# wooginawunan/multi-modal-uncertainty

Hardware: AMD Instinct MI355X
Metric: image+text samples/sec/node, MMBT Food-101 bs=256 seq=512; ECE/NLL parity (higher is better)
Workload: dtype bf16

## Files before the change

### multi-modal-uncertainty_amd/csrc/gemm.hip

```cpp
#include "mmu_common.h"
#include "mmu_internal.h"
#include <cstdlib>

namespace mmu {

constexpr int BKT = 64;

#ifdef MMU_GEMM_STAMPS
__device__ uint64_t g_gemm_stamps[1 << 16][4];
#define GEMM_STAMP(i)                                                                       \
  do {                                                                                      \
    if (threadIdx.x == 0) {                                                                 \
      const int lin_ = (int)(blockIdx.x + gridDim.x * (blockIdx.y + gridDim.y * blockIdx.z)); \
      if (lin_ < (1 << 16)) g_gemm_stamps[lin_][i] = __builtin_amdgcn_s_memtime();          \
    }                                                                                       \
  } while (0)
#else
#define GEMM_STAMP(i) \
  do {                \
  } while (0)
#endif

static __device__ __forceinline__ int sw_mn(int r) { return (r & 7) ^ (((r >> 3) & 1) << 2); }

static __device__ __forceinline__ void tile_of(int pid, int tiles_m, int tiles_n, int group_m, int& tm, int& tn) {
  const int per_group = group_m * tiles_n;
  const int g = pid / per_group, first = g * group_m;
  const int gm = tiles_m - first < group_m ? tiles_m - first : group_m;
  const int r = pid - g * per_group;
  tm = first + r % gm;
  tn = r / gm;
}
static __device__ __forceinline__ void block_tile(const GemmParams& p, int64_t& z, int& slice, int& tm, int& tn) {
  const int ntiles = p.tiles_m * p.tiles_n;
  const int per_z = ntiles * (int)gridDim.y;
  const int lin = (int)(blockIdx.x + gridDim.x * (blockIdx.y + gridDim.y * blockIdx.z));
  const int pid = xcd_remap(lin, per_z * (int)gridDim.z);
  z = pid / per_z;
  const int r = pid - (int)z * per_z;
  slice = r / ntiles;
  tile_of(r - slice * ntiles, p.tiles_m, p.tiles_n, p.group_m, tm, tn);
}

template <bool KMAJ, int ROWB>
static __device__ __forceinline__ bf16x8 s_frag(const char* s, int row0, int ks, int l) {
  if (KMAJ) {
    const int row = row0 + (l & 15), c = 4 * ks + (l >> 4);
    return *(const bf16x8*)(s + row * 128 + ((c ^ (row & 7)) << 4));
  } else {
    const int g = l >> 4, i = l & 15, q = i >> 2, p = i & 3;
    const int b = row0 >> 4;
    const int k0 = 32 * ks + 8 * g + q, k1 = k0 + 4;
    const char* a0 = s + k0 * ROWB + ((b ^ sw_mn(k0)) << 5) + 8 * p;
    const char* a1 = s + k1 * ROWB + ((b ^ sw_mn(k1)) << 5) + 8 * p;
    bf16x4 lo = __builtin_amdgcn_ds_read_tr16_b64_v4bf16((MMU_LDS(bf16x4)*)a0);
    bf16x4 hi = __builtin_amdgcn_ds_read_tr16_b64_v4bf16((MMU_LDS(bf16x4)*)a1);
    return __builtin_shufflevector(lo, hi, 0, 1, 2, 3, 4, 5, 6, 7);
  }
}


template <int EPI, bool OUT_F32>
static __device__ __forceinline__ void epi_oct(const GemmParams& p, void* cdst, bf16* xdst, uint64_t qd,
                                               float (&v)[8], const float (&in)[8], float scale, uint32_t thr,
                                               uint64_t seed) {
  if (EPI == MMU_EPI_BIAS_GELU) {
    float d[8];
#pragma unroll
    for (int r = 0; r < 8; ++r) gelu_pair(v[r], v[r], d[r]);
    if (xdst) {
      bf16x8 o;
#pragma unroll
      for (int r = 0; r < 8; ++r) o[r] = f2bf(d[r]);
      *(bf16x8*)xdst = o;
    }
  } else if (EPI == MMU_EPI_BIAS_DROP_RES) {
    if (thr) {
      const uint32_t keep = mmu_keep4(seed, qd, thr) | (mmu_keep4(seed, qd + 1, thr) << 4);
#pragma unroll
      for (int r = 0; r < 8; ++r) v[r] = ((keep >> r) & 1) ? v[r] * scale : 0.f;
    }
#pragma unroll
    for (int r = 0; r < 8; ++r) v[r] += in[r];
  } else if (EPI == MMU_EPI_BIAS_DROP_QGELU) {
    uint32_t keep = 0xFFu;
    if (thr) keep = mmu_keep4(seed, qd, thr) | (mmu_keep4(seed, qd + 1, thr) << 4);
    float d[8];
#pragma unroll
    for (int r = 0; r < 8; ++r) {
      const float kz = ((keep >> r) & 1) ? scale : 0.f;
      const float u = v[r] * kz;
      const float sg = __builtin_amdgcn_rcpf(1.0f + __builtin_amdgcn_exp2f(u * -2.4554669595930157f));
      v[r] = u * sg;
      d[r] = kz * fmaf(1.702f * u * sg, 1.0f - sg, sg);
    }
    if (xdst) {
      bf16x8 o;
#pragma unroll
      for (int r = 0; r < 8; ++r) o[r] = f2bf(d[r]);
      *(bf16x8*)xdst = o;
    }
  } else if (EPI == MMU_EPI_DGELU) {
#pragma unroll
    for (int r = 0; r < 8; ++r) v[r] *= in[r];
  } else if (EPI == MMU_EPI_ADD_RES) {
#pragma unroll
    for (int r = 0; r < 8; ++r) v[r] += in[r];
  }
  if (OUT_F32) {
    float4* C = (float4*)cdst;
    float4 lo = make_float4(v[0], v[1], v[2], v[3]), hi = make_float4(v[4], v[5], v[6], v[7]);
// ... 382 lines not shown
    const char* sb = sa + SBM * BKT * 2;
    const bool more = kt + 1 < nk;
    if (more) {
      const int64_t k1 = kb + (int64_t)(kt + 1) * BKT;
      conva_g_load(ra, p.A, p, cr, k1, t);
      g_load<true>(rb, p.B, p.ldb, n0, p.N, k1, ke, t);
    }
#pragma unroll
    for (int ks = 0; ks < 2; ++ks) {
      bf16x8 fb[4], fa[4];
#pragma unroll
      for (int i = 0; i < 4; ++i) fb[i] = s_frag<true, 256>(sb, 64 * wn + 16 * i, ks, l);
#pragma unroll
      for (int j = 0; j < 4; ++j) fa[j] = s_frag<true, 256>(sa, 64 * wm + 16 * j, ks, l);
#pragma unroll
      for (int i = 0; i < 4; ++i)
#pragma unroll
        for (int j = 0; j < 4; ++j)
          acc[i][j] = __builtin_amdgcn_mfma_f32_16x16x32_bf16(fb[i], fa[j], acc[i][j], 0, 0, 0);
    }
    if (more) {
      char* dst = smem + ((kt + 1) & 1) * S_STAGE;
      s_store<true>(dst, ra, t);
      s_store<true>(dst + SBM * BKT * 2, rb, t);
    }
    __syncthreads();
  }
  epilogue_block<EPI, false, 4>(p, z, slice, m0 + 64 * wm, n0 + 64 * wn, acc, l, smem + w * 16384);
}

constexpr int BBM = 256, BBN = 256;
constexpr int B_TILE = BBM * BKT * 2;
constexpr int B_STAGE = 2 * B_TILE;

template <bool KMAJ>
static __device__ __forceinline__ void dma_tile(char* s, __amdgpu_buffer_rsrc_t rsrc, int64_t ld, int64_t r0,
                                                int64_t k0, int w, int l) {
#pragma unroll
  for (int i = 0; i < 4; ++i) {
    const int piece = w * 4 + i;
    uint32_t src;
    if (KMAJ) {
      const int row = piece * 8 + (l >> 3), c = (l & 7) ^ (row & 7);
      src = (uint32_t)(((r0 + row) * ld + k0 + 8 * c) * 2);
    } else {
      const int kr = piece * 2 + (l >> 5), j = l & 31;
      const int b = (j >> 1) ^ sw_mn(kr);
      src = (uint32_t)(((k0 + kr) * ld + r0 + 16 * b + 8 * (j & 1)) * 2);
    }
    __builtin_amdgcn_raw_ptr_buffer_load_lds(rsrc, (MMU_LDS(void)*)(s + piece * 1024), 16, src, 0, 0, 0);
  }
}

static __device__ __forceinline__ void dma_tile_convb(char* s, __amdgpu_buffer_rsrc_t rsrc, const GemmParams& p,
                                                      int dh, int dw, int64_t ci0, int64_t k0, int w, int l) {
  const int H = p.conv_h, W = p.conv_w, C = p.conv_c, s_ = p.conv_s;
  const int Wo = p.conv_wo, HW = p.conv_ho * Wo;
  const float rhw = 1.0f / (float)HW, rw = 1.0f / (float)Wo;
#pragma unroll
  for (int i = 0; i < 4; ++i) {
    const int piece = w * 4 + i;
    const int kr = piece * 2 + (l >> 5), j = l & 31;
    const int b = (j >> 1) ^ sw_mn(kr);
    const int pix = (int)k0 + kr;
    int img = (int)((float)pix * rhw);
    int rem = pix - img * HW;
    if (rem < 0) { --img; rem += HW; } else if (rem >= HW) { ++img; rem -= HW; }
    int hh = (int)((float)rem * rw);
    int ww = rem - hh * Wo;
    if (ww < 0) { --hh; ww += Wo; } else if (ww >= Wo) { ++hh; ww -= Wo; }
    hh = hh * s_ + dh;
    ww = ww * s_ + dw;
    const bool ok = pix < p.K && (unsigned)hh < (unsigned)H && (unsigned)ww < (unsigned)W;
    const uint32_t src = ok ? (uint32_t)(((((int64_t)img * H + hh) * W + ww) * C + ci0 + 16 * b + 8 * (j & 1)) * 2)
                            : 0x7FFFFFF0u;
    __builtin_amdgcn_raw_ptr_buffer_load_lds(rsrc, (MMU_LDS(void)*)(s + piece * 1024), 16, src, 0, 0, 0);
  }
}

struct ConvRows {
  int base[4], h[4], w[4];
};
static __device__ __forceinline__ ConvRows conv_rows_init(const GemmParams& p, int64_t m0, int w, int l) {
  ConvRows r;
  const int Wo = p.conv_wo, HWo = p.conv_ho * Wo;
#pragma unroll
  for (int i = 0; i < 4; ++i) {
    const int row = (w * 4 + i) * 8 + (l >> 3);
    const int64_t pix = m0 + row;
    const int img = (int)(pix / HWo), rem = (int)(pix - (int64_t)img * HWo);
    const int ho = rem / Wo;
    r.base[i] = pix < p.M ? img * p.conv_h : -1;
    r.h[i] = ho * p.conv_s - p.conv_pad;
    r.w[i] = (rem - ho * Wo) * p.conv_s - p.conv_pad;
  }
  return r;
}
static __device__ __forceinline__ void dma_tile_conva(char* s, __amdgpu_buffer_rsrc_t rsrc, const GemmParams& p,
                                                      const ConvRows& r, int64_t k0, int w, int l) {
  const int H = p.conv_h, W = p.conv_w, C = p.conv_c;
  const int tap = (int)(k0 / C), ci0 = (int)(k0 - (int64_t)tap * C);
  const int dh = tap / p.conv_ks, dw = tap - dh * p.conv_ks;
#pragma unroll
  for (int i = 0; i < 4; ++i) {
    const int piece = w * 4 + i;
    const int row = piece * 8 + (l >> 3), c = (l & 7) ^ (row & 7);
    const int hh = r.h[i] + dh, ww = r.w[i] + dw;
    const bool ok = r.base[i] >= 0 && (unsigned)hh < (unsigned)H && (unsigned)ww < (unsigned)W && k0 < p.K;
    const uint32_t src = ok ? (uint32_t)((((int64_t)(r.base[i] + hh) * W + ww) * C + ci0 + 8 * c) * 2) : 0x7FFFFFF0u;
    __builtin_amdgcn_raw_ptr_buffer_load_lds(rsrc, (MMU_LDS(void)*)(s + piece * 1024), 16, src, 0, 0, 0);
  }
}

template <bool AK, bool BKM, int EPI, bool OUT_F32, int GATHER>
static __device__ __forceinline__ void gemm_big_body(const GemmParams& p) {
  __shared__ __attribute__((aligned(16))) char smem[2 * B_STAGE];
  const int t = threadIdx.x, l = t & 63;
  const int w = __builtin_amdgcn_readfirstlane(t >> 6);
  const int wm = w >> 2, wn = w & 3;
  int tm, tn, slice;
  int64_t z;
  GEMM_STAMP(0);
  block_tile(p, z, slice, tm, tn);
  const int64_t m0 = (int64_t)tm * BBM, n0 = (int64_t)tn * BBN;
  const int64_t a_bytes = GATHER == 2 ? p.conv_in_bytes : (AK ? p.M * p.lda : p.K * p.lda) * 2;
  const int64_t b_bytes = GATHER == 1 ? p.conv_in_bytes : (BKM ? p.N * p.ldb : p.K * p.ldb) * 2;
  const __amdgpu_buffer_rsrc_t ra =
      __builtin_amdgcn_make_buffer_rsrc((void*)(p.A + z * p.sA), 0, (int)(uint32_t)a_bytes, 0x00020000);
  const __amdgpu_buffer_rsrc_t rb =
      __builtin_amdgcn_make_buffer_rsrc((void*)(p.B + z * p.sB), 0, (int)(uint32_t)b_bytes, 0x00020000);

  f32x4 acc[4][8];
#pragma unroll
  for (int i = 0; i < 4; ++i)
#pragma unroll
    for (int j = 0; j < 8; ++j) acc[i][j] = f32x4{0.f, 0.f, 0.f, 0.f};

  const int64_t kb = (int64_t)slice * p.kchunk;
  const int64_t ke = kb + p.kchunk < p.K ? kb + p.kchunk : p.K;
  const int nk = (int)((ke - kb + BKT - 1) / BKT);
  const int tap = GATHER == 1 ? (int)(n0 / p.conv_c) : 0;
  const int dh = GATHER == 1 ? tap / p.conv_ks - p.conv_pad : 0;
  const int dw = GATHER == 1 ? tap % p.conv_ks - p.conv_pad : 0;
  const int64_t ci0 = GATHER == 1 ? n0 - (int64_t)tap * p.conv_c : 0;
  auto dma_b = [&](char* d, int64_t k) {
    if (GATHER == 1) dma_tile_convb(d, rb, p, dh, dw, ci0, k, w, l);
    else dma_tile<BKM>(d, rb, p.ldb, n0, k, w, l);
  };
  ConvRows crow;
  if (GATHER == 2) crow = conv_rows_init(p, m0, w, l);
  auto dma_a = [&](char* d, int64_t k) {
    if (GATHER == 2) dma_tile_conva(d, ra, p, crow, k, w, l);
    else dma_tile<AK>(d, ra, p.lda, m0, k, w, l);
  };
  dma_a(smem, kb);
  dma_b(smem + B_TILE, kb);
  asm volatile("s_waitcnt vmcnt(0)" ::: "memory");
  __syncthreads();
  GEMM_STAMP(1);
  for (int kt = 0; kt < nk; ++kt) {
    const char* sa = smem + (kt & 1) * B_STAGE;
    const char* sb = sa + B_TILE;
    if (kt + 1 < nk) {
      char* d = smem + ((kt + 1) & 1) * B_STAGE;
      const int64_t k1 = kb + (int64_t)(kt + 1) * BKT;
      dma_a(d, k1);
      dma_b(d + B_TILE, k1);
    }
#pragma unroll
    for (int ks = 0; ks < 2; ++ks) {
      bf16x8 fb[4], fa[8];
#pragma unroll
      for (int i = 0; i < 4; ++i) fb[i] = s_frag<BKM, 512>(sb, 64 * wn + 16 * i, ks, l);
#pragma unroll
      for (int j = 0; j < 8; ++j) fa[j] = s_frag<AK, 512>(sa, 128 * wm + 16 * j, ks, l);
#pragma unroll
      for (int i = 0; i < 4; ++i)
#pragma unroll
        for (int j = 0; j < 8; ++j)
          acc[i][j] = __builtin_amdgcn_mfma_f32_16x16x32_bf16(fb[i], fa[j], acc[i][j], 0, 0, 0);
    }
    asm volatile("s_waitcnt vmcnt(0)" ::: "memory");
    __syncthreads();
  }
  GEMM_STAMP(2);
  epilogue_block<EPI, OUT_F32, 8>(p, z, slice, m0 + 128 * wm, n0 + 64 * wn, acc, l, smem + w * 16384);
#ifdef MMU_GEMM_STAMPS
  asm volatile("s_waitcnt vmcnt(0)" ::: "memory");
#endif
  GEMM_STAMP(3);
}

template <bool AK, bool BKM, int EPI, bool OUT_F32>
__global__ __launch_bounds__(512) void gemm_big_kernel(GemmParams p) {
  gemm_big_body<AK, BKM, EPI, OUT_F32, 0>(p);
}

__global__ __launch_bounds__(512) void gemm_convw_kernel(GemmParams p) {
  gemm_big_body<false, false, MMU_EPI_STORE, true, 1>(p);
}

template <int EPI>
__global__ __launch_bounds__(512) void gemm_conva_kernel(GemmParams p) {
  gemm_big_body<true, true, EPI, false, 2>(p);
}

constexpr int WBM = 256, WBN = 384;
constexpr int W_TA = WBM * BKT * 2;
constexpr int W_TB = WBN * BKT * 2;
constexpr int W_STAGE = W_TA + W_TB;

template <int P>
static __device__ __forceinline__ void dma_kmaj(char* s, __amdgpu_buffer_rsrc_t rsrc, int64_t ld, int64_t r0,
                                                int64_t k0, int w, int l) {
#pragma unroll
  for (int i = 0; i < P; ++i) {
    const int piece = w * P + i;
    const int row = piece * 8 + (l >> 3), c = (l & 7) ^ (row & 7);
    const uint32_t src = (uint32_t)(((r0 + row) * ld + k0 + 8 * c) * 2);
    __builtin_amdgcn_raw_ptr_buffer_load_lds(rsrc, (MMU_LDS(void)*)(s + piece * 1024), 16, src, 0, 0, 0);
  }
}

template <int EPI, bool OUT_F32>
__global__ __launch_bounds__(512) void gemm_wide_kernel(GemmParams p) {
  __shared__ __attribute__((aligned(16))) char smem[2 * W_STAGE];
  const int t = threadIdx.x, l = t & 63;
  const int w = __builtin_amdgcn_readfirstlane(t >> 6);
  const int wm = w >> 1, wn = w & 1;
  int tm, tn, slice;
  int64_t z;
  block_tile(p, z, slice, tm, tn);
  const int64_t m0 = (int64_t)tm * WBM, n0 = (int64_t)tn * WBN;
  const __amdgpu_buffer_rsrc_t ra =
      __builtin_amdgcn_make_buffer_rsrc((void*)(p.A + z * p.sA), 0, (int)(uint32_t)(p.M * p.lda * 2), 0x00020000);
  const __amdgpu_buffer_rsrc_t rb =
      __builtin_amdgcn_make_buffer_rsrc((void*)(p.B + z * p.sB), 0, (int)(uint32_t)(p.N * p.ldb * 2), 0x00020000);
  f32x4 acc[3][4][4];
#pragma unroll
  for (int c = 0; c < 3; ++c)
#pragma unroll
    for (int i = 0; i < 4; ++i)
#pragma unroll
      for (int j = 0; j < 4; ++j) acc[c][i][j] = f32x4{0.f, 0.f, 0.f, 0.f};
  const int nk = (int)(p.K / BKT);
  dma_kmaj<4>(smem, ra, p.lda, m0, 0, w, l);
  dma_kmaj<6>(smem + W_TA, rb, p.ldb, n0, 0, w, l);
  asm volatile("s_waitcnt vmcnt(0)" ::: "memory");
  __syncthreads();
  for (int kt = 0; kt < nk; ++kt) {
    const char* sa = smem + (kt & 1) * W_STAGE;
// ... 541 lines not shown
```

### multi-modal-uncertainty_amd/csrc/attention.hip

```cpp
#include "mmu_common.h"
#include "mmu_internal.h"
#include <cstdlib>
#include <type_traits>
#include <utility>

namespace mmu {

constexpr float LOG2E = 1.4426950408889634f;
constexpr float LN2 = 0.6931471805599453f;
constexpr float NEG_INF = -__builtin_huge_valf();

static __device__ __forceinline__ uint32_t lowbias32(uint32_t x) {
  x ^= x >> 16; x *= 0x7feb352du; x ^= x >> 15; x *= 0x846ca68bu; x ^= x >> 16;
  return x;
}
static __device__ __forceinline__ uint32_t seed_for(uint64_t seed, int bh) {
  return lowbias32((uint32_t)seed ^ lowbias32((uint32_t)(seed >> 32) + 0x9E3779B9u * (uint32_t)(bh + 1)));
}
static __device__ __forceinline__ uint32_t drop_pair(uint32_t sbh, uint32_t q, uint32_t key, uint32_t Lp) {
  return lowbias32(((q * Lp + key) >> 1) ^ sbh);
}

static __device__ __forceinline__ float max3f(float a, float b, float c) {
  return __builtin_fmaxf(__builtin_fmaxf(a, b), c);
}
static __device__ __forceinline__ uint32_t bfi(uint32_t m, uint32_t a, uint32_t b) {
  return (m & a) | (~m & b);
}
static __device__ __forceinline__ uint32_t keepmask(uint32_t w, uint32_t pos) {
  uint32_t r;
  asm("v_bfe_i32 %0, %1, %2, 1" : "=v"(r) : "v"(w), "v"(pos));
  return r;
}
template <typename F, int... R>
static __device__ __forceinline__ void static_for(F&& f, std::integer_sequence<int, R...>) {
  (f(std::integral_constant<int, R>{}), ...);
}
template <int POS>
static __device__ __forceinline__ uint32_t keepmask(uint32_t w) {
  uint32_t r;
  asm("v_bfe_i32 %0, %1, %2, 1" : "=v"(r) : "v"(w), "n"(POS));
  return r;
}
static __host__ __device__ __forceinline__ uint32_t drop_thr(float p) { return (uint32_t)(p * 65536.0f + 0.5f); }

static __device__ __forceinline__ int fsw(int r) { return (((r >> 1) & 1) << 2) | ((r >> 3) & 3); }
static __device__ __forceinline__ int tile_off(int row, int chunk) { return row * 128 + ((chunk ^ fsw(row)) << 4); }

static __device__ __forceinline__ bf16x8 row_frag(const char* s, int row0, int ks, int l) {
  return *(const bf16x8*)(s + tile_off(row0 + (l & 31), 2 * ks + (l >> 5)));
}
static __device__ __forceinline__ bf16x8 tr_frag(const char* s, int row0, int col0, int l) {
  const int g = l >> 4, i = l & 15, q = i >> 2, p = i & 3, h = g >> 1;
  const int col = col0 + 16 * (g & 1) + 4 * p;
  const int r0 = row0 + 4 * h + q, r1 = r0 + 8;
  const int cb = col * 2;
  const char* a0 = s + tile_off(r0, cb >> 4) + (cb & 15);
  const char* a1 = s + tile_off(r1, cb >> 4) + (cb & 15);
  bf16x4 lo = __builtin_amdgcn_ds_read_tr16_b64_v4bf16((MMU_LDS(bf16x4)*)a0);
  bf16x4 hi = __builtin_amdgcn_ds_read_tr16_b64_v4bf16((MMU_LDS(bf16x4)*)a1);
  return __builtin_shufflevector(lo, hi, 0, 1, 2, 3, 4, 5, 6, 7);
}
static __device__ __forceinline__ bf16x8 acc_frag(const f32x16& a, int s) {
  bf16x8 r;
#pragma unroll
  for (int j = 0; j < 8; ++j) r[j] = f2bf(a[8 * s + j]);
  return r;
}
static __device__ __forceinline__ bf16x8 scale_frag(uint4 u, float sc) {
  bf16x8 v = *(bf16x8*)&u;
#pragma unroll
  for (int j = 0; j < 8; ++j) v[j] = f2bf(bf2f(v[j]) * sc);
  return v;
}

static __device__ __forceinline__ __amdgpu_buffer_rsrc_t urs(const void* base, int bytes) {
  const uint64_t a = (uint64_t)base;
  const uint32_t lo = __builtin_amdgcn_readfirstlane((uint32_t)a);
  const uint32_t hi = __builtin_amdgcn_readfirstlane((uint32_t)(a >> 32));
  const int n = __builtin_amdgcn_readfirstlane(bytes);
  return __builtin_amdgcn_make_buffer_rsrc((void*)(((uint64_t)hi << 32) | lo), 0, n, 0x00020000);
}

static __device__ __forceinline__ void dma16(__amdgpu_buffer_rsrc_t r, char* lds, uint32_t off) {
  __builtin_amdgcn_raw_ptr_buffer_load_lds(r, (MMU_LDS(void)*)lds, 16, off, 0, 0, 0);
}
static __device__ __forceinline__ __amdgpu_buffer_rsrc_t urs_at(const void* base, int bytes, int off) {
  return urs((const char*)base + off, bytes > off ? bytes - off : 0);
}
static __device__ __forceinline__ void dma4(__amdgpu_buffer_rsrc_t r, char* lds, uint32_t off) {
  __builtin_amdgcn_raw_ptr_buffer_load_lds(r, (MMU_LDS(void)*)lds, 4, off, 0, 0, 0);
}
static __device__ __forceinline__ void raw_barrier() {
  __builtin_amdgcn_s_barrier();
  asm volatile("" ::: "memory");
}

static __device__ __forceinline__ void block_coords(int& bx, int& bh) {
  const int gx = gridDim.x;
  const int wid = xcd_remap(blockIdx.y * gx + blockIdx.x, gx * gridDim.y);
  bh = wid / gx;
  bx = wid - bh * gx;
}

constexpr int FWD_NS = 2;
constexpr int FWD_TILE = 64 * 128;
constexpr int FWD_STAGE = 2 * FWD_TILE + 256;
constexpr int FWD_MAX_NKV = 9;

constexpr float DEFER_LOG2 = 8.0f;
constexpr uint32_t kDropMul24[8] = {0x9E3779u, 0x85EBCBu, 0xC2B2AFu, 0xA7D4EBu,
                                    0x965667u, 0xD3A265u, 0xFD7047u, 0xB55A4Fu};

static __device__ __forceinline__ uint32_t pair_draw(uint32_t hb, int i) {
  const uint32_t src = i ? __builtin_amdgcn_alignbit(hb, hb, 4 * i) : hb;
// ... 312 lines not shown
      const __amdgpu_buffer_rsrc_t rt = urs_at(do_base, do_bytes, q0 * p.ld_do * 2);
#pragma unroll
      for (int pc = 0; pc < 4; ++pc) dma16(rt, st + DK_TILE + pc * 1024, pc_off[pc]);
      dma4(urs_at(k_base, drop ? L * nkv * 8 : 0, q0 * nkv * 8), st + 2 * DK_TILE + 256, kw_off);
    }
  };
  auto wait_for = [&](int ahead) {
    if (w == 0) {
      if (ahead >= 2) asm volatile("s_waitcnt vmcnt(12)" ::: "memory");
      else if (ahead == 1) asm volatile("s_waitcnt vmcnt(6)" ::: "memory");
      else asm volatile("s_waitcnt vmcnt(0)" ::: "memory");
    } else {
      if (ahead >= 2) asm volatile("s_waitcnt vmcnt(10)" ::: "memory");
      else if (ahead == 1) asm volatile("s_waitcnt vmcnt(5)" ::: "memory");
      else asm volatile("s_waitcnt vmcnt(0)" ::: "memory");
    }
  };
  asm volatile("s_waitcnt vmcnt(0)" ::: "memory");
  for (int i = 0; i < DK_NS - 1 && i < nq; ++i) issue(i);
  auto qtile = [&](int i, auto sg_tag) {
    constexpr int SG = decltype(sg_tag)::value;
    const int ahead = nq - 1 - i < DK_NS - 2 ? nq - 1 - i : DK_NS - 2;
    wait_for(ahead);
    raw_barrier();
    if (i + DK_NS - 1 < nq) issue(i + DK_NS - 1);
    const char* st = smem + SG * DK_STAGE;
    const char* Qs = st;
    const char* Ds = st + DK_TILE;
    const float* lse = (const float*)(st + 2 * DK_TILE);
    const float* dlt = lse + 32;
    const uint32_t* kbit = (const uint32_t*)(st + 2 * DK_TILE + 256) + w;
    if (wave_live) {
      f32x4 l4[4], nd4[4];
      uint32_t kwr[16];
#pragma unroll
      for (int j = 0; j < 4; ++j) {
        l4[j] = *(const f32x4*)(lse + 8 * j + 4 * h);
        nd4[j] = *(const f32x4*)(dlt + 8 * j + 4 * h);
        if (DROP)
#pragma unroll
          for (int i2 = 0; i2 < 4; ++i2) kwr[4 * j + i2] = kbit[2 * (8 * j + 4 * h + i2)];
      }
      f32x16 sc, dp;
#pragma unroll
      for (int r = 0; r < 16; ++r) {
        sc[r] = l4[r >> 2][r & 3];
        dp[r] = nd4[r >> 2][r & 3];
      }
#pragma unroll
      for (int ks = 0; ks < 4; ++ks) {
        sc = __builtin_amdgcn_mfma_f32_32x32x16_bf16(row_frag(Qs, 0, ks, l), kf[ks], sc, 0, 0, 0);
        dp = __builtin_amdgcn_mfma_f32_32x32x16_bf16(row_frag(Ds, 0, ks, l), vf[ks], dp, 0, 0, 0);
      }
      f32x16 pz;
#pragma unroll
      for (int r = 0; r < 16; ++r) {
        const float pr = __builtin_amdgcn_exp2f(fmaf(sc[r], -LOG2E, mkey));
        if (DROP) {
          const uint32_t m = keepmask(kwr[r], lane31);
          pz[r] = __uint_as_float(m & __float_as_uint(pr));
          sc[r] = pr * __uint_as_float(bfi(m, __float_as_uint(dp[r]), __float_as_uint(nd4[r >> 2][r & 3])));
        } else {
          pz[r] = pr;
          sc[r] = pr * dp[r];
        }
      }
#pragma unroll
      for (int s2 = 0; s2 < 2; ++s2) {
        if (s2 == 1 && 32 * i + 16 >= L) break;
        bf16x8 pf = acc_frag(pz, s2), sf = acc_frag(sc, s2);
#pragma unroll
        for (int dt = 0; dt < 2; ++dt) {
          dv[dt] = __builtin_amdgcn_mfma_f32_32x32x16_bf16(pf, tr_frag(Ds, 16 * s2, 32 * dt, l), dv[dt], 0, 0, 0);
          dk[dt] = __builtin_amdgcn_mfma_f32_32x32x16_bf16(sf, tr_frag(Qs, 16 * s2, 32 * dt, l), dk[dt], 0, 0, 0);
        }
      }
    }
  };
  for (int i0 = 0; i0 < nq; i0 += DK_NS) {
    qtile(i0, std::integral_constant<int, 0>{});
    if (i0 + 1 < nq) qtile(i0 + 1, std::integral_constant<int, 1>{});
    if (i0 + 2 < nq) qtile(i0 + 2, std::integral_constant<int, 2>{});
    if (i0 + 3 < nq) qtile(i0 + 3, std::integral_constant<int, 3>{});
  }
  static_assert(DK_NS == 4, "the dK/dV loop is unrolled by its ring depth");
  const float dks = 0.125f * zs;
  if (p.colsum) {
    float* red = (float*)smem;
    raw_barrier();
#pragma unroll
    for (int dt = 0; dt < 2; ++dt) {
      float sk = 0.f, sv = 0.f;
#pragma unroll
      for (int r = 0; r < 16; ++r) {
        const bool ok = k0w + (r & 3) + 8 * (r >> 2) + 4 * h < L;
        sk += ok ? dk[dt][r] : 0.f;
        sv += ok ? dv[dt][r] : 0.f;
      }
      sk += __shfl_xor(sk, 32, 64);
      sv += __shfl_xor(sv, 32, 64);
      if (h == 0) {
        red[w * 128 + 32 * dt + l] = sk * dks;
        red[w * 128 + 64 + 32 * dt + l] = sv * zs;
      }
    }
    raw_barrier();
    if (t < 128) {
      const int nqb = (L + 127) / 128, nkb = (L + 63) / 64, B = p.batch;
      const float v = red[t] + red[128 + t];
      const int64_t row = (int64_t)nqb * B + (t < 64 ? 0 : (int64_t)nkb * B) + (int64_t)bx * B + b;
      p.colsum[row * HD + hd * 64 + (t & 63)] = v;
    }
  }
  if (!wave_live) return;
  bf16* outb = p.out + (int64_t)b * L * p.ld_out + hd * 64;
#pragma unroll
  for (int dt = 0; dt < 2; ++dt)
#pragma unroll
    for (int r = 0; r < 16; ++r) {
      const int kk = k0w + (r & 3) + 8 * (r >> 2) + 4 * h;
      if (kk < L) {
        const int64_t off = (int64_t)kk * p.ld_out + 32 * dt + (l & 31);
        outb[off + HD] = f2bf(dk[dt][r] * dks);
        outb[off + 2 * HD] = f2bf(dv[dt][r] * zs);
      }
    }
}
// ... 41 lines not shown
      const bf16x8 ov = *(bf16x8*)&u;
#pragma unroll
      for (int e = 0; e < 8; ++e) dsum = fmaf(bf2f(ov[e]), bf2f(df[ks][e]), dsum);
    }
    dsum += __shfl_xor(dsum, 32, 64);
    if (qv && h == 0) p.delta[(int64_t)bh * L + q] = -dsum / zs;
  }
  const float nlse2 = qv ? -p.lse[(int64_t)bh * L + q] * LOG2E : -__builtin_huge_valf();
  const float ndz = -dsum / zs;
  const uint32_t ndz_bits = __float_as_uint(ndz);
  f32x16 dq[2];
#pragma unroll
  for (int i = 0; i < 16; ++i) { dq[0][i] = 0.f; dq[1][i] = 0.f; }

  uint32_t kv_off[4];
#pragma unroll
  for (int pc = 0; pc < 4; ++pc) {
    const int piece = 4 * (w & 1) + pc;
    const int row = 8 * piece + (l >> 3), c = (l & 7) ^ fsw(row);
    kv_off[pc] = (uint32_t)((row * p.ld_qkv + (w < 2 ? HD : 2 * HD) + hd * 64 + 8 * c) * 2);
  }
  const uint32_t m_off = (uint32_t)(16 * l), kw_off = (uint32_t)(((q0w + (l >> 1)) * nkv * 8) + 4 * (l & 1));
  auto issue = [&](int j) {
    char* st = smem + (j % DQ_NS) * DQ_STAGE;
    const int k0 = j * 64;
    char* dst = st + (w < 2 ? 0 : DQ_TILE);
    const __amdgpu_buffer_rsrc_t rt = urs_at(kv_base, kv_bytes, k0 * p.ld_qkv * 2);
#pragma unroll
    for (int pc = 0; pc < 4; ++pc) dma16(rt, dst + (4 * (w & 1) + pc) * 1024, kv_off[pc]);
    if (w == 0 && l < 16) dma16(urs_at(m_base, L * 4, k0 * 4), st + 2 * DQ_TILE, m_off);
    dma4(urs_at(k_base, k_bytes, j * 8), st + 2 * DQ_TILE + 256 + w * 256, kw_off);
  };
  auto wait_for = [&](int ahead) {
    if (w == 0) {
      if (ahead >= 1) asm volatile("s_waitcnt vmcnt(6)" ::: "memory");
      else asm volatile("s_waitcnt vmcnt(0)" ::: "memory");
    } else {
      if (ahead >= 1) asm volatile("s_waitcnt vmcnt(5)" ::: "memory");
      else asm volatile("s_waitcnt vmcnt(0)" ::: "memory");
    }
  };
  asm volatile("s_waitcnt vmcnt(0)" ::: "memory");
  for (int j = 0; j < DQ_NS - 1 && j < nkv; ++j) issue(j);
  auto tile_step = [&](int j, auto sg_tag) {
    constexpr int SG = decltype(sg_tag)::value;
    const int ahead = nkv - 1 - j < DQ_NS - 2 ? nkv - 1 - j : DQ_NS - 2;
    wait_for(ahead);
    raw_barrier();
    if (j + DQ_NS - 1 < nkv) issue(j + DQ_NS - 1);
    const char* st = smem + SG * DQ_STAGE;
    const char* Ks = st;
    const char* Vs = st + DQ_TILE;
    const float* mk = (const float*)(st + 2 * DQ_TILE);
    const uint32_t* kwords = (const uint32_t*)(st + 2 * DQ_TILE + 256 + w * 256);
    if (wave_live) {
      const uint64_t kw = drop ? ((uint64_t)kwords[2 * (l & 31) + 1] << 32 | kwords[2 * (l & 31)]) : ~0ull;
      const uint64_t kwh = kw >> (4 * h);
#pragma unroll
      for (int st2 = 0; st2 < 2; ++st2) {
        if (st2 == 1 && 64 * j + 32 >= L) break;
        const uint32_t kw32 = (uint32_t)(kwh >> (32 * st2));
        f32x16 sc, dp;
#pragma unroll
        for (int g = 0; g < 4; ++g) {
          const f32x4 mv = *(const f32x4*)(mk + 32 * st2 + 8 * g + 4 * h);
#pragma unroll
          for (int e = 0; e < 4; ++e) {
            sc[4 * g + e] = mv[e];
            dp[4 * g + e] = ndz;
          }
        }
#pragma unroll
        for (int ks = 0; ks < 4; ++ks) {
          sc = __builtin_amdgcn_mfma_f32_32x32x16_bf16(row_frag(Ks, 32 * st2, ks, l), qf[ks], sc, 0, 0, 0);
          dp = __builtin_amdgcn_mfma_f32_32x32x16_bf16(row_frag(Vs, 32 * st2, ks, l), df[ks], dp, 0, 0, 0);
        }
        auto one = [&](auto r_tag) {
          constexpr int r = decltype(r_tag)::value;
          const float pr = __builtin_amdgcn_exp2f(fmaf(sc[r], LOG2E, nlse2));
          const uint32_t m = keepmask<(r & 3) + 8 * (r >> 2)>(kw32);
          sc[r] = pr * __uint_as_float(bfi(m, __float_as_uint(dp[r]), ndz_bits));
        };
        static_for(one, std::make_integer_sequence<int, 16>{});
#pragma unroll
        for (int s2 = 0; s2 < 2; ++s2) {
          bf16x8 sf = acc_frag(sc, s2);
#pragma unroll
          for (int dt = 0; dt < 2; ++dt)
            dq[dt] = __builtin_amdgcn_mfma_f32_32x32x16_bf16(tr_frag(Ks, 32 * st2 + 16 * s2, 32 * dt, l), sf, dq[dt],
                                                             0, 0, 0);
        }
      }
    }
    };
  for (int j0 = 0; j0 < nkv; j0 += DQ_NS) {
    tile_step(j0, std::integral_constant<int, 0>{});
    if (j0 + 1 < nkv) tile_step(j0 + 1, std::integral_constant<int, 1>{});
    if (j0 + 2 < nkv) tile_step(j0 + 2, std::integral_constant<int, 2>{});
  }
  if (p.colsum) {
    constexpr int RS = 68;
    static_assert(4 * 32 * RS * 4 <= DQ_NS * DQ_STAGE, "dQ column-sum rows exceed the ring's LDS");
    float* rows = (float*)smem;
    raw_barrier();
    float* mine = rows + w * 32 * RS + (l & 31) * RS;
    const float sc = qv ? 0.125f * zs : 0.f;
#pragma unroll
    for (int dt = 0; dt < 2; ++dt)
#pragma unroll
      for (int g = 0; g < 4; ++g)
        *(float4*)(mine + 32 * dt + 8 * g + 4 * h) =
            make_float4(dq[dt][4 * g] * sc, dq[dt][4 * g + 1] * sc, dq[dt][4 * g + 2] * sc, dq[dt][4 * g + 3] * sc);
    raw_barrier();
    if (t < 64) {
      float v = 0.f;
      for (int r = 0; r < 128; ++r) v += rows[r * RS + t];
      p.colsum[((int64_t)bx * p.batch + b) * HD + hd * 64 + t] = v;
    }
  }
  if (!qv) return;
  bf16* ob = p.out + ((int64_t)b * L + q) * p.ld_out + hd * 64;
#pragma unroll
  for (int dt = 0; dt < 2; ++dt)
#pragma unroll
    for (int g = 0; g < 4; ++g) {
      const float s = 0.125f * zs;
      bf16x4 v = {f2bf(dq[dt][4 * g] * s), f2bf(dq[dt][4 * g + 1] * s), f2bf(dq[dt][4 * g + 2] * s),
                  f2bf(dq[dt][4 * g + 3] * s)};
      *(bf16x4*)(ob + 32 * dt + 8 * g + 4 * h) = v;
    }
}

void attention_bwd_launch(const AttnParams& p, hipStream_t s) {
  hipLaunchKernelGGL(attn_dq_dma_kernel, dim3((p.L + 127) / 128, p.batch * p.heads), dim3(256), 0, s, p);
  if (drop_thr(p.drop_p))
    hipLaunchKernelGGL(attn_dkdv_dma_kernel<true>, dim3((p.L + 63) / 64, p.batch * p.heads), dim3(128), 0, s, p);
  else
    hipLaunchKernelGGL(attn_dkdv_dma_kernel<false>, dim3((p.L + 63) / 64, p.batch * p.heads), dim3(128), 0, s, p);
}

constexpr int R0_GROUPS = 32;

static __device__ __forceinline__ void ld8f(const bf16* p, float (&o)[8]) {
  const uint4 u = *(const uint4*)p;
  const bf16x8 v = *(const bf16x8*)&u;
// ... 200 lines not shown
```

### multi-modal-uncertainty_amd/csrc/mmu_common.h

```cpp
#pragma once
#include <hip/hip_runtime.h>
#include <stdint.h>

typedef __bf16 bf16;
typedef __bf16 bf16x8 __attribute__((ext_vector_type(8)));
typedef __bf16 bf16x4 __attribute__((ext_vector_type(4)));
typedef float f32x4 __attribute__((ext_vector_type(4)));
typedef float f32x2 __attribute__((ext_vector_type(2)));
typedef float f32x16 __attribute__((ext_vector_type(16)));
typedef uint16_t u16x4 __attribute__((ext_vector_type(4)));
typedef uint16_t u16x8 __attribute__((ext_vector_type(8)));

#define MMU_LDS(T) __attribute__((address_space(3))) T

static __device__ __forceinline__ float bf2f(bf16 x) { return (float)x; }
static __device__ __forceinline__ bf16 f2bf(float x) { return (bf16)x; }

static __device__ __forceinline__ uint32_t mmu_lowbias32(uint32_t x) {
  x ^= x >> 16; x *= 0x7feb352du; x ^= x >> 15; x *= 0x846ca68bu; x ^= x >> 16;
  return x;
}
static __device__ __forceinline__ uint32_t mmu_seed32(uint64_t seed) {
  return mmu_lowbias32((uint32_t)seed ^ mmu_lowbias32((uint32_t)(seed >> 32) ^ 0x68bc21ebu));
}
static __device__ __forceinline__ uint32_t mmu_keep4(uint64_t seed, uint64_t quad, uint32_t thr16) {
  const uint32_t x = (((uint32_t)quad << 1) ^ ((uint32_t)(quad >> 31) * 0x9E3779B8u)) ^ mmu_seed32(seed);
  const uint32_t h0 = mmu_lowbias32(x), h1 = mmu_lowbias32(x ^ 1u);
  return ((h0 & 0xFFFFu) >= thr16 ? 1u : 0u) | ((h0 >> 16) >= thr16 ? 2u : 0u) |
         ((h1 & 0xFFFFu) >= thr16 ? 4u : 0u) | ((h1 >> 16) >= thr16 ? 8u : 0u);
}
static __device__ __forceinline__ uint64_t mmu_eff_seed(uint64_t seed, const uint64_t* off) {
  return off ? seed ^ (*off * 0x9E3779B97F4A7C15ull) : seed;
}
static __device__ __forceinline__ bool mmu_keep1(uint64_t seed, uint64_t idx, uint32_t thr16) {
  const uint64_t quad = idx >> 2;
  const uint32_t x = (((uint32_t)quad << 1) ^ ((uint32_t)(quad >> 31) * 0x9E3779B8u)) ^ mmu_seed32(seed);
  const uint32_t h = mmu_lowbias32(x ^ (uint32_t)((idx >> 1) & 1));
  return ((h >> (16 * (idx & 1))) & 0xFFFFu) >= thr16;
}

static __device__ __forceinline__ void gelu_pair(float z, float& g, float& dg) {
  const float t = __builtin_amdgcn_rcpf(fmaf(0.3275911f * 0.70710678118654752f, fabsf(z), 1.0f));
  float P = fmaf(0.5f * 1.061405429f, t, 0.5f * -1.453152027f);
  P = fmaf(P, t, 0.5f * 1.421413741f);
  P = fmaf(P, t, 0.5f * -0.284496736f);
  P = fmaf(P, t, 0.5f * 0.254829592f);
  const float e = __builtin_amdgcn_exp2f(z * z * -0.72134752044448170f);
  const float h = (t * P) * e;
  const float phi = z >= 0.f ? 1.0f - h : h;
  g = z * phi;
  dg = fmaf(z * 0.39894228040143268f, e, phi);
}
static __device__ __forceinline__ float gelu_erf(float z) {
  float g, dg;
  gelu_pair(z, g, dg);
  return g;
}

static __device__ __forceinline__ float wave_sum(float v) {
#pragma unroll
  for (int o = 32; o > 0; o >>= 1) v += __shfl_xor(v, o, 64);
  return v;
}
static __device__ __forceinline__ float wave_max(float v) {
#pragma unroll
  for (int o = 32; o > 0; o >>= 1) v = fmaxf(v, __shfl_xor(v, o, 64));
  return v;
}

// ... 5 lines not shown
```

Before: 1690.

## Precompute MN-major DMA and LDS fragment offsets, cap VGPRs for wgrad GEMMs

For the MN-major f32-output store GEMM variants (weight-gradient and conv weight-gradient), per-lane DMA source offsets and LDS fragment base addresses are computed once outside the K loop. Each iteration then adds a scalar K offset, or XORs a fragment index into the base, instead of redoing the swizzle arithmetic. The conv-B gather column swizzle is also hoisted. The aim is to cut VALU address math and register pressure so the wgrad kernels fit under a 96-VGPR cap and gain occupancy, at the risk of spills given the 128 fp32 accumulators per lane.

```diff
diff --git a/multi-modal-uncertainty_amd/csrc/gemm.hip b/multi-modal-uncertainty_amd/csrc/gemm.hip
--- a/multi-modal-uncertainty_amd/csrc/gemm.hip
+++ b/multi-modal-uncertainty_amd/csrc/gemm.hip
@@ -57,6 +57,19 @@
     bf16x4 hi = __builtin_amdgcn_ds_read_tr16_b64_v4bf16((MMU_LDS(bf16x4)*)a1);
     return __builtin_shufflevector(lo, hi, 0, 1, 2, 3, 4, 5, 6, 7);
   }
+}
+
+static __device__ __forceinline__ uint32_t mn_frag_base(int R0, int l) {
+  const int i = l & 15, k0 = 8 * (l >> 4) + (i >> 2);
+  return (uint32_t)(k0 * 512 + (((R0 >> 4) ^ sw_mn(k0)) << 5) + 8 * (i & 3));
+}
+static __device__ __forceinline__ bf16x8 mn_frag(const char* smem, uint32_t base, int f, int ks) {
+  const MMU_LDS(char)* s = (const MMU_LDS(char)*)smem;
+  const uint32_t a0 = (base ^ (uint32_t)(f << 5)) + 16384 * ks;
+  const uint32_t a1 = (base ^ (uint32_t)((f ^ 4) << 5)) + 16384 * ks + 2048;
+  bf16x4 lo = __builtin_amdgcn_ds_read_tr16_b64_v4bf16((MMU_LDS(bf16x4)*)(s + a0));
+  bf16x4 hi = __builtin_amdgcn_ds_read_tr16_b64_v4bf16((MMU_LDS(bf16x4)*)(s + a1));
+  return __builtin_shufflevector(lo, hi, 0, 1, 2, 3, 4, 5, 6, 7);
 }
 
 
@@ -545,16 +558,30 @@
   }
 }
 
+static __device__ __forceinline__ uint32_t dma_mn_lane(int64_t ld, int64_t r0, int w, int l, int i) {
+  const int kr = (w * 4 + i) * 2 + (l >> 5), j = l & 31;
+  const int b = (j >> 1) ^ sw_mn(kr);
+  return (uint32_t)((kr * ld + r0 + 16 * b + 8 * (j & 1)) * 2);
+}
+static __device__ __forceinline__ void dma_tile_mn(char* s, __amdgpu_buffer_rsrc_t rsrc, const uint32_t (&inv)[4],
+                                                   uint32_t kofs, int w) {
+#pragma unroll
+  for (int i = 0; i < 4; ++i)
+    __builtin_amdgcn_raw_ptr_buffer_load_lds(rsrc, (MMU_LDS(void)*)(s + (w * 4 + i) * 1024), 16, inv[i] + kofs, 0, 0, 0);
+}
+
 static __device__ __forceinline__ void dma_tile_convb(char* s, __amdgpu_buffer_rsrc_t rsrc, const GemmParams& p,
                                                       int dh, int dw, int64_t ci0, int64_t k0, int w, int l) {
   const int H = p.conv_h, W = p.conv_w, C = p.conv_c, s_ = p.conv_s;
   const int Wo = p.conv_wo, HW = p.conv_ho * Wo;
   const float rhw = 1.0f / (float)HW, rw = 1.0f / (float)Wo;
+  const int j = l & 31;
+  int col0 = 16 * ((j >> 1) ^ (l >> 5) ^ ((w & 1) << 2)) + 8 * (j & 1);
+  asm volatile("" : "+v"(col0));
 #pragma unroll
   for (int i = 0; i < 4; ++i) {
     const int piece = w * 4 + i;
-    const int kr = piece * 2 + (l >> 5), j = l & 31;
-    const int b = (j >> 1) ^ sw_mn(kr);
+    const int kr = piece * 2 + (l >> 5);
     const int pix = (int)k0 + kr;
     int img = (int)((float)pix * rhw);
     int rem = pix - img * HW;
@@ -565,7 +592,7 @@
     hh = hh * s_ + dh;
     ww = ww * s_ + dw;
     const bool ok = pix < p.K && (unsigned)hh < (unsigned)H && (unsigned)ww < (unsigned)W;
-    const uint32_t src = ok ? (uint32_t)(((((int64_t)img * H + hh) * W + ww) * C + ci0 + 16 * b + 8 * (j & 1)) * 2)
+    const uint32_t src = ok ? (uint32_t)(((((int64_t)img * H + hh) * W + ww) * C + ci0 + (col0 ^ (32 * i))) * 2)
                             : 0x7FFFFFF0u;
     __builtin_amdgcn_raw_ptr_buffer_load_lds(rsrc, (MMU_LDS(void)*)(s + piece * 1024), 16, src, 0, 0, 0);
   }
@@ -636,14 +663,30 @@
   const int dh = GATHER == 1 ? tap / p.conv_ks - p.conv_pad : 0;
   const int dw = GATHER == 1 ? tap % p.conv_ks - p.conv_pad : 0;
   const int64_t ci0 = GATHER == 1 ? n0 - (int64_t)tap * p.conv_c : 0;
+  constexpr bool LEAN = !AK && !BKM && EPI == MMU_EPI_STORE && OUT_F32;
+  uint32_t inv_a[4], inv_b[4];
+  if (LEAN) {
+#pragma unroll
+    for (int i = 0; i < 4; ++i) {
+      inv_a[i] = dma_mn_lane(p.lda, m0, w, l, i);
+      inv_b[i] = GATHER == 0 ? dma_mn_lane(p.ldb, n0, w, l, i) : 0;
+    }
+  }
+  auto k_ofs = [](int64_t k, int64_t ld) {
+    uint32_t o = (uint32_t)(k * ld * 2);
+    asm volatile("" : "+s"(o));
+    return o;
+  };
   auto dma_b = [&](char* d, int64_t k) {
     if (GATHER == 1) dma_tile_convb(d, rb, p, dh, dw, ci0, k, w, l);
+    else if (LEAN) dma_tile_mn(d, rb, inv_b, k_ofs(k, p.ldb), w);
     else dma_tile<BKM>(d, rb, p.ldb, n0, k, w, l);
   };
   ConvRows crow;
   if (GATHER == 2) crow = conv_rows_init(p, m0, w, l);
   auto dma_a = [&](char* d, int64_t k) {
     if (GATHER == 2) dma_tile_conva(d, ra, p, crow, k, w, l);
+    else if (LEAN) dma_tile_mn(d, ra, inv_a, k_ofs(k, p.lda), w);
     else dma_tile<AK>(d, ra, p.lda, m0, k, w, l);
   };
   dma_a(smem, kb);
@@ -651,6 +694,8 @@
   asm volatile("s_waitcnt vmcnt(0)" ::: "memory");
   __syncthreads();
   GEMM_STAMP(1);
+  const uint32_t base_a = LEAN ? mn_frag_base(128 * wm, l) : 0;
+  const uint32_t base_b = LEAN ? mn_frag_base(64 * wn, l) + B_TILE : 0;
   for (int kt = 0; kt < nk; ++kt) {
     const char* sa = smem + (kt & 1) * B_STAGE;
     const char* sb = sa + B_TILE;
@@ -660,13 +705,15 @@
       dma_a(d, k1);
       dma_b(d + B_TILE, k1);
     }
+    uint32_t oa = base_a + (kt & 1) * B_STAGE, ob = base_b + (kt & 1) * B_STAGE;
+    if (LEAN) asm volatile("" : "+v"(oa), "+v"(ob));
 #pragma unroll
     for (int ks = 0; ks < 2; ++ks) {
       bf16x8 fb[4], fa[8];
 #pragma unroll
-      for (int i = 0; i < 4; ++i) fb[i] = s_frag<BKM, 512>(sb, 64 * wn + 16 * i, ks, l);
-#pragma unroll
-      for (int j = 0; j < 8; ++j) fa[j] = s_frag<AK, 512>(sa, 128 * wm + 16 * j, ks, l);
+      for (int i = 0; i < 4; ++i) fb[i] = LEAN ? mn_frag(smem, ob, i, ks) : s_frag<BKM, 512>(sb, 64 * wn + 16 * i, ks, l);
+#pragma unroll
+      for (int j = 0; j < 8; ++j) fa[j] = LEAN ? mn_frag(smem, oa, j, ks) : s_frag<AK, 512>(sa, 128 * wm + 16 * j, ks, l);
 #pragma unroll
       for (int i = 0; i < 4; ++i)
 #pragma unroll
@@ -689,7 +736,13 @@
   gemm_big_body<AK, BKM, EPI, OUT_F32, 0>(p);
 }
 
-__global__ __launch_bounds__(512) void gemm_convw_kernel(GemmParams p) {
+#define MMU_WGRAD_VGPRS __attribute__((amdgpu_num_vgpr(96)))
+template <>
+__global__ __launch_bounds__(512) MMU_WGRAD_VGPRS void gemm_big_kernel<false, false, MMU_EPI_STORE, true>(GemmParams p) {
+  gemm_big_body<false, false, MMU_EPI_STORE, true, 0>(p);
+}
+
+__global__ __launch_bounds__(512) MMU_WGRAD_VGPRS void gemm_convw_kernel(GemmParams p) {
   gemm_big_body<false, false, MMU_EPI_STORE, true, 1>(p);
 }
 
```

Measured after the change: 1695 (median of 6 runs). No clear change (+0.3%).

## Issue transposed LDS reads early via inline asm and overlap with MFMA

Applied to the files above, without the earlier changes.

Adds inline-asm LDS transposed-read helpers with compile-time offsets and explicit lgkmcnt waits. The attention backward dK/dV and dQ loops now issue these reads before the softmax/exp math and wait only right before the MFMAs that consume them, so LDS latency is hidden behind ALU work. The big GEMM k-step is restructured the same way: all fragment loads are issued up front and then consumed one at a time with staged waitcnts and sched barriers. The cost is more live VGPRs and hand-managed waitcnt counts, which break silently if the compiler reorders or inserts other LDS ops.

```diff
diff --git a/multi-modal-uncertainty_amd/csrc/attention.hip b/multi-modal-uncertainty_amd/csrc/attention.hip
--- a/multi-modal-uncertainty_amd/csrc/attention.hip
+++ b/multi-modal-uncertainty_amd/csrc/attention.hip
@@ -61,6 +61,21 @@
   bf16x4 hi = __builtin_amdgcn_ds_read_tr16_b64_v4bf16((MMU_LDS(bf16x4)*)a1);
   return __builtin_shufflevector(lo, hi, 0, 1, 2, 3, 4, 5, 6, 7);
 }
+struct TrPair {
+  bf16x4 lo, hi;
+};
+template <int BASE, int ROW0, int COL0>
+static __device__ __forceinline__ TrPair tr_issue(const char* s, int l) {
+  const int g = l >> 4, i = l & 15, q = i >> 2, p = i & 3, h = g >> 1;
+  const int cb = (COL0 + 16 * (g & 1) + 4 * p) * 2;
+  const int rl = 4 * h + q;
+  const char* r = s + rl * 128 + (cb & 15);
+  TrPair t;
+  t.lo = lds_tr16<BASE + ROW0 * 128>(r + (((cb >> 4) ^ fsw(ROW0 + rl)) << 4));
+  t.hi = lds_tr16<BASE + (ROW0 + 8) * 128>(r + (((cb >> 4) ^ fsw(ROW0 + 8 + rl)) << 4));
+  return t;
+}
+static __device__ __forceinline__ bf16x8 tr_get(const TrPair& t) { return lds_landed(t.lo, t.hi); }
 static __device__ __forceinline__ bf16x8 acc_frag(const f32x16& a, int s) {
   bf16x8 r;
 #pragma unroll
@@ -479,6 +494,16 @@
         sc = __builtin_amdgcn_mfma_f32_32x32x16_bf16(row_frag(Qs, 0, ks, l), kf[ks], sc, 0, 0, 0);
         dp = __builtin_amdgcn_mfma_f32_32x32x16_bf16(row_frag(Ds, 0, ks, l), vf[ks], dp, 0, 0, 0);
       }
+      constexpr int QB = SG * DK_STAGE, DB = SG * DK_STAGE + DK_TILE;
+      TrPair dt_[2][2], qt_[2][2];
+      dt_[0][0] = tr_issue<DB, 0, 0>(smem, l);
+      qt_[0][0] = tr_issue<QB, 0, 0>(smem, l);
+      dt_[0][1] = tr_issue<DB, 0, 32>(smem, l);
+      qt_[0][1] = tr_issue<QB, 0, 32>(smem, l);
+      dt_[1][0] = tr_issue<DB, 16, 0>(smem, l);
+      qt_[1][0] = tr_issue<QB, 16, 0>(smem, l);
+      dt_[1][1] = tr_issue<DB, 16, 32>(smem, l);
+      qt_[1][1] = tr_issue<QB, 16, 32>(smem, l);
       f32x16 pz;
 #pragma unroll
       for (int r = 0; r < 16; ++r) {
@@ -492,14 +517,15 @@
           sc[r] = pr * dp[r];
         }
       }
+      lds_wait<0>();
 #pragma unroll
       for (int s2 = 0; s2 < 2; ++s2) {
         if (s2 == 1 && 32 * i + 16 >= L) break;
         bf16x8 pf = acc_frag(pz, s2), sf = acc_frag(sc, s2);
 #pragma unroll
         for (int dt = 0; dt < 2; ++dt) {
-          dv[dt] = __builtin_amdgcn_mfma_f32_32x32x16_bf16(pf, tr_frag(Ds, 16 * s2, 32 * dt, l), dv[dt], 0, 0, 0);
-          dk[dt] = __builtin_amdgcn_mfma_f32_32x32x16_bf16(sf, tr_frag(Qs, 16 * s2, 32 * dt, l), dk[dt], 0, 0, 0);
+          dv[dt] = __builtin_amdgcn_mfma_f32_32x32x16_bf16(pf, tr_get(dt_[s2][dt]), dv[dt], 0, 0, 0);
+          dk[dt] = __builtin_amdgcn_mfma_f32_32x32x16_bf16(sf, tr_get(qt_[s2][dt]), dk[dt], 0, 0, 0);
         }
       }
     }
@@ -647,14 +673,17 @@
     const char* Ks = st;
     const char* Vs = st + DQ_TILE;
     const float* mk = (const float*)(st + 2 * DQ_TILE);
-    const uint32_t* kwords = (const uint32_t*)(st + 2 * DQ_TILE + 256 + w * 256);
     if (wave_live) {
-      const uint64_t kw = drop ? ((uint64_t)kwords[2 * (l & 31) + 1] << 32 | kwords[2 * (l & 31)]) : ~0ull;
-      const uint64_t kwh = kw >> (4 * h);
-#pragma unroll
-      for (int st2 = 0; st2 < 2; ++st2) {
-        if (st2 == 1 && 64 * j + 32 >= L) break;
-        const uint32_t kw32 = (uint32_t)(kwh >> (32 * st2));
+      uint64_t kw_raw = lds_read64<SG * DQ_STAGE + 2 * DQ_TILE + 256>(smem + w * 256 + 8 * (l & 31));
+      uint64_t kwh = 0;
+      auto half = [&](auto st2_tag) {
+        constexpr int st2 = decltype(st2_tag)::value;
+        if (st2 == 1 && 64 * j + 32 >= L) return;
+        TrPair kt[2][2];
+        kt[0][0] = tr_issue<SG * DQ_STAGE, 32 * st2, 0>(smem, l);
+        kt[0][1] = tr_issue<SG * DQ_STAGE, 32 * st2, 32>(smem, l);
+        kt[1][0] = tr_issue<SG * DQ_STAGE, 32 * st2 + 16, 0>(smem, l);
+        kt[1][1] = tr_issue<SG * DQ_STAGE, 32 * st2 + 16, 32>(smem, l);
         f32x16 sc, dp;
 #pragma unroll
         for (int g = 0; g < 4; ++g) {
@@ -670,6 +699,9 @@
           sc = __builtin_amdgcn_mfma_f32_32x32x16_bf16(row_frag(Ks, 32 * st2, ks, l), qf[ks], sc, 0, 0, 0);
           dp = __builtin_amdgcn_mfma_f32_32x32x16_bf16(row_frag(Vs, 32 * st2, ks, l), df[ks], dp, 0, 0, 0);
         }
+        lds_wait<0>();
+        if (st2 == 0) kwh = (drop ? lds_landed64(kw_raw) : ~0ull) >> (4 * h);
+        const uint32_t kw32 = (uint32_t)(kwh >> (32 * st2));
         auto one = [&](auto r_tag) {
           constexpr int r = decltype(r_tag)::value;
           const float pr = __builtin_amdgcn_exp2f(fmaf(sc[r], LOG2E, nlse2));
@@ -682,10 +714,11 @@
           bf16x8 sf = acc_frag(sc, s2);
 #pragma unroll
           for (int dt = 0; dt < 2; ++dt)
-            dq[dt] = __builtin_amdgcn_mfma_f32_32x32x16_bf16(tr_frag(Ks, 32 * st2 + 16 * s2, 32 * dt, l), sf, dq[dt],
-                                                             0, 0, 0);
+            dq[dt] = __builtin_amdgcn_mfma_f32_32x32x16_bf16(tr_get(kt[s2][dt]), sf, dq[dt], 0, 0, 0);
         }
-      }
+      };
+      half(std::integral_constant<int, 0>{});
+      half(std::integral_constant<int, 1>{});
     }
     };
   for (int j0 = 0; j0 < nkv; j0 += DQ_NS) {
diff --git a/multi-modal-uncertainty_amd/csrc/gemm.hip b/multi-modal-uncertainty_amd/csrc/gemm.hip
--- a/multi-modal-uncertainty_amd/csrc/gemm.hip
+++ b/multi-modal-uncertainty_amd/csrc/gemm.hip
@@ -1,10 +1,13 @@
 #include "mmu_common.h"
 #include "mmu_internal.h"
 #include <cstdlib>
+#include <type_traits>
 
 namespace mmu {
 
 constexpr int BKT = 64;
+template <int N>
+using ic = std::integral_constant<int, N>;
 
 #ifdef MMU_GEMM_STAMPS
 __device__ uint64_t g_gemm_stamps[1 << 16][4];
@@ -56,6 +59,74 @@
     bf16x4 lo = __builtin_amdgcn_ds_read_tr16_b64_v4bf16((MMU_LDS(bf16x4)*)a0);
     bf16x4 hi = __builtin_amdgcn_ds_read_tr16_b64_v4bf16((MMU_LDS(bf16x4)*)a1);
     return __builtin_shufflevector(lo, hi, 0, 1, 2, 3, 4, 5, 6, 7);
+  }
+}
+
+template <int ROWB, int KS, int BASE>
+static __device__ __forceinline__ void s_frag_tr_issue(const char* s, int row0, int l, bf16x4& lo, bf16x4& hi) {
+  const int g = l >> 4, i = l & 15, q = i >> 2, p = i & 3;
+  const int b = row0 >> 4;
+  const int k0 = 8 * g + q;
+  const char* r = s + k0 * ROWB + 8 * p;
+  lo = lds_tr16<BASE + 32 * KS * ROWB>(r + ((b ^ sw_mn(k0)) << 5));
+  hi = lds_tr16<BASE + (32 * KS + 4) * ROWB>(r + ((b ^ sw_mn(k0) ^ 4) << 5));
+}
+
+template <bool AK, bool BKM, int KS>
+static __device__ __forceinline__ void big_kstep(const char* sa, int wm, int wn, int l, f32x4 (&acc)[4][8]) {
+  constexpr int B_OFF = 256 * BKT * 2;
+  bf16x8 fb[4], fa[8];
+  if constexpr (AK && BKM) {
+#pragma unroll
+    for (int i = 0; i < 4; ++i) fb[i] = s_frag<true, 512>(sa + B_OFF, 64 * wn + 16 * i, KS, l);
+#pragma unroll
+    for (int j = 0; j < 8; ++j) fa[j] = s_frag<true, 512>(sa, 128 * wm + 16 * j, KS, l);
+#pragma unroll
+    for (int i = 0; i < 4; ++i)
+#pragma unroll
+      for (int j = 0; j < 8; ++j)
+        acc[i][j] = __builtin_amdgcn_mfma_f32_16x16x32_bf16(fb[i], fa[j], acc[i][j], 0, 0, 0);
+  } else {
+    bf16x4 blo[4], bhi[4], alo[8], ahi[8];
+    if constexpr (!BKM) {
+#pragma unroll
+      for (int i = 0; i < 4; ++i) s_frag_tr_issue<512, KS, B_OFF>(sa, 64 * wn + 16 * i, l, blo[i], bhi[i]);
+    } else {
+#pragma unroll
+      for (int i = 0; i < 4; ++i) fb[i] = s_frag<true, 512>(sa + B_OFF, 64 * wn + 16 * i, KS, l);
+    }
+    if constexpr (!AK) {
+#pragma unroll
+      for (int j = 0; j < 8; ++j) s_frag_tr_issue<512, KS, 0>(sa, 128 * wm + 16 * j, l, alo[j], ahi[j]);
+      auto step = [&](auto jc, auto nc) {
+        constexpr int j = decltype(jc)::value;
+        lds_wait<decltype(nc)::value>();
+        if constexpr (j == 0 && !BKM) {
+#pragma unroll
+          for (int i = 0; i < 4; ++i) fb[i] = lds_landed(blo[i], bhi[i]);
+        }
+        fa[j] = lds_landed(alo[j], ahi[j]);
+#pragma unroll
+        for (int i = 0; i < 4; ++i)
+          acc[i][j] = __builtin_amdgcn_mfma_f32_16x16x32_bf16(fb[i], fa[j], acc[i][j], 0, 0, 0);
+        __builtin_amdgcn_sched_barrier(0);
+      };
+      step(ic<0>{}, ic<14>{}); step(ic<1>{}, ic<12>{}); step(ic<2>{}, ic<10>{}); step(ic<3>{}, ic<8>{});
+      step(ic<4>{}, ic<6>{});  step(ic<5>{}, ic<4>{});  step(ic<6>{}, ic<2>{});  step(ic<7>{}, ic<0>{});
+    } else {
+#pragma unroll
+      for (int j = 0; j < 8; ++j) fa[j] = s_frag<true, 512>(sa, 128 * wm + 16 * j, KS, l);
+      auto step = [&](auto icn, auto nc) {
+        constexpr int i = decltype(icn)::value;
+        lds_wait<decltype(nc)::value>();
+        fb[i] = lds_landed(blo[i], bhi[i]);
+#pragma unroll
+        for (int j = 0; j < 8; ++j)
+          acc[i][j] = __builtin_amdgcn_mfma_f32_16x16x32_bf16(fb[i], fa[j], acc[i][j], 0, 0, 0);
+        __builtin_amdgcn_sched_barrier(0);
+      };
+      step(ic<0>{}, ic<6>{}); step(ic<1>{}, ic<4>{}); step(ic<2>{}, ic<2>{}); step(ic<3>{}, ic<0>{});
+    }
   }
 }
 
@@ -653,26 +724,14 @@
   GEMM_STAMP(1);
   for (int kt = 0; kt < nk; ++kt) {
     const char* sa = smem + (kt & 1) * B_STAGE;
-    const char* sb = sa + B_TILE;
     if (kt + 1 < nk) {
       char* d = smem + ((kt + 1) & 1) * B_STAGE;
       const int64_t k1 = kb + (int64_t)(kt + 1) * BKT;
       dma_a(d, k1);
       dma_b(d + B_TILE, k1);
     }
-#pragma unroll
-    for (int ks = 0; ks < 2; ++ks) {
-      bf16x8 fb[4], fa[8];
-#pragma unroll
-      for (int i = 0; i < 4; ++i) fb[i] = s_frag<BKM, 512>(sb, 64 * wn + 16 * i, ks, l);
-#pragma unroll
-      for (int j = 0; j < 8; ++j) fa[j] = s_frag<AK, 512>(sa, 128 * wm + 16 * j, ks, l);
-#pragma unroll
-      for (int i = 0; i < 4; ++i)
-#pragma unroll
-        for (int j = 0; j < 8; ++j)
-          acc[i][j] = __builtin_amdgcn_mfma_f32_16x16x32_bf16(fb[i], fa[j], acc[i][j], 0, 0, 0);
-    }
+    big_kstep<AK, BKM, 0>(sa, wm, wn, l, acc);
+    big_kstep<AK, BKM, 1>(sa, wm, wn, l, acc);
     asm volatile("s_waitcnt vmcnt(0)" ::: "memory");
     __syncthreads();
   }
diff --git a/multi-modal-uncertainty_amd/csrc/mmu_common.h b/multi-modal-uncertainty_amd/csrc/mmu_common.h
--- a/multi-modal-uncertainty_amd/csrc/mmu_common.h
+++ b/multi-modal-uncertainty_amd/csrc/mmu_common.h
@@ -15,6 +15,31 @@
 
 static __device__ __forceinline__ float bf2f(bf16 x) { return (float)x; }
 static __device__ __forceinline__ bf16 f2bf(float x) { return (bf16)x; }
+
+template <int OFF>
+static __device__ __forceinline__ bf16x4 lds_tr16(const char* a) {
+  bf16x4 r;
+  asm volatile("ds_read_b64_tr_b16 %0, %1 offset:%2" : "=v"(r) : "v"((MMU_LDS(const char)*)a), "n"(OFF));
+  return r;
+}
+template <int N>
+static __device__ __forceinline__ void lds_wait() {
+  asm volatile("s_waitcnt lgkmcnt(%0)" ::"n"(N));
+}
+template <int OFF>
+static __device__ __forceinline__ uint64_t lds_read64(const char* a) {
+  uint64_t r;
+  asm volatile("ds_read_b64 %0, %1 offset:%2" : "=v"(r) : "v"((MMU_LDS(const char)*)a), "n"(OFF));
+  return r;
+}
+static __device__ __forceinline__ uint64_t lds_landed64(uint64_t v) {
+  asm volatile("" : "+v"(v));
+  return v;
+}
+static __device__ __forceinline__ bf16x8 lds_landed(bf16x4 lo, bf16x4 hi) {
+  asm volatile("" : "+v"(lo), "+v"(hi));
+  return __builtin_shufflevector(lo, hi, 0, 1, 2, 3, 4, 5, 6, 7);
+}
 
 static __device__ __forceinline__ uint32_t mmu_lowbias32(uint32_t x) {
   x ^= x >> 16; x *= 0x7feb352du; x ^= x >> 15; x *= 0x846ca68bu; x ^= x >> 16;
```

Result: faster. 1712 before, 1760 after (median of 6 runs) (+2.8%).
